# Hongje/OTVM

Measured on AMD Instinct MI355X. Metric: frames_per_sec, higher is better.
Workload: dtype f16x3 (fp32 operands split into fp16 hi+lo, fp32 accumulate); 1 GPU; synthetic 1920x1080 clip, T=140 frames (untimed lead-in 0 + warmup 5 + timed: the last 135), memory every 5, max 5 slots, trimap propagation + alpha + memorize per frame, one sequence per GPU; weights=synthetic (otvm_amd.synth_weights seed 0), parallelism=sequence-per-gpu x1, batch=1

## Files before the change

### include/otvm_hip.h

```cpp
#ifndef OTVM_HIP_H
#define OTVM_HIP_H

#include <stdint.h>

#ifdef __cplusplus
extern "C" {
#endif

#define OTVM_ACT_NONE 0
#define OTVM_ACT_RELU 1
#define OTVM_ACT_LEAKY 2

#define OTVM_PREC_F32 0
#define OTVM_PREC_F16X3 1
#define OTVM_PREC_F16 2

const char* otvm_last_error(void);
#define OTVM_ABI_VERSION 21
int otvm_abi_version(void);

int otvm_pack_conv_weight(const float* w_oihw, int O, int I, int kh, int kw, int ws, const float* scale,
                          float* w_packed, int O_pad, int I_pad, int K_pad, void* stream);

int64_t otvm_patch_weight_bytes_f16x3(int O, int I_pad);
// ... 25 lines not shown
    int tune;
    void* splitk_ws; int64_t splitk_ws_bytes;
    int batch;
    int64_t in_bs, out_bs, res_bs;
    int gn_bs;
    int norm_bs;
    const void* w_wfrag;
    const float* gn_gamma; const float* gn_beta;
    float* gn_scale_out; float* gn_shift_out;
    unsigned* gn_counter;
    int gn_tab_bs;
    int ws_bs;
    const float* res_scale;
    int res_scale_bs;
    const float* in_res; int in_res_ld; int64_t in_res_bs;
} otvm_conv_params;
int otvm_conv2d_accepts_input_residual(const otvm_conv_params* p);

typedef struct otvm_head_params {
    const float* w; const float* b; int n_out;
    const float* img; int img_ld;
    int64_t P;
    float* alpha_out; int alpha_stride;
    float* tri_out;
    float* sm; int sm_ld;
    int64_t img_bs, alpha_bs, tri_bs, sm_bs;
    const void* w16;
} otvm_head_params;
int otvm_conv2d_head(const otvm_conv_params* p, const otvm_head_params* h, void* stream);
int otvm_conv2d_head_fgr(const otvm_conv_params* p, const otvm_head_params* h, float* fgr, int64_t fgr_bs, void* stream);
// ... 249 lines not shown
```

### otvm_amd/csrc/conv_f16x3.hip

```cpp
#include "common.h"
#include <type_traits>
#include <hip/hip_fp16.h>
#include <stdlib.h>

#include "conv_f16x3_kernel.h"

namespace {

#ifndef OTVM_WAVE_PF
#define OTVM_WAVE_PF 3
#endif

template <bool RELU_IN>
__global__ __launch_bounds__(64) void conv_wave_f16x3_kernel(const Conv3Args pa) {
    Conv3Args p = pa;
    {
        const int zb = blockIdx.z;
        p.in += zb * p.in_bs;
        p.out += zb * p.out_bs;
        if (p.residual) p.residual += zb * p.res_bs;
        if (p.gn_stats) p.gn_stats += zb * p.gn_bs;
        p.wscale += zb * p.ws_bs;
        if (p.bias) p.bias += zb * p.ws_bs;
    }
// ... 325 lines not shown
    return 0;
}

extern "C" int64_t otvm_wave_weight_bytes_f16x3(int O_pad, int K_pad) { return (int64_t)O_pad * K_pad * 2 * sizeof(_Float16); }

extern "C" int otvm_pack_wave_weight_f16x3(const void* w_hi, const void* w_lo, int O_pad, int K_pad, void* w_wfrag, void* stream) {
    OTVM_REQUIRE(w_hi && w_lo && w_wfrag && O_pad % 32 == 0 && K_pad % 32 == 0, "otvm_pack_wave_weight_f16x3: bad arguments");
    hipLaunchKernelGGL(pack_wave_weight_kernel, dim3(O_pad / 32), dim3(256), 0, (hipStream_t)stream, (const _Float16*)w_hi,
                       (const _Float16*)w_lo, K_pad, (_Float16*)w_wfrag);
    OTVM_CHECK_LAUNCH("otvm_pack_wave_weight_f16x3");
    return 0;
}

int otvm_conv2d_patch_f16x3_impl(const otvm_conv_params* p, void* stream);

static inline int tune_code(int tile, int S) { return (tile + 1) * 16 + S; }

static int launch_wave(Conv3Args& a, hipStream_t s, int ksplit) {
    a.tiles_m = otvm_ceil_div(a.M, 64);
    a.tiles_n = otvm_ceil_div(a.Cout, 64);
    const dim3 grid(a.tiles_m * a.tiles_n, ksplit, a.batch), block(64);
    if ((int64_t)a.H * a.W * a.in_ld >= (1ll << 31) - (1 << 20)) {
        otvm_set_error("otvm_conv2d(f16x3 wave tile): input view too large for 32-bit offsets");
        return 1;
    }
    if (a.in_relu) hipLaunchKernelGGL((conv_wave_f16x3_kernel<true>), grid, block, 0, s, a);
    else hipLaunchKernelGGL((conv_wave_f16x3_kernel<false>), grid, block, 0, s, a);
    OTVM_CHECK_LAUNCH("otvm_conv2d(f16x3 wave tile)");
    return 0;
}

static int launch_tile(int tile, Conv3Args& a, hipStream_t s, int S) {
    if (a.npass == 1) return otvm_launch_tile_p1(tile, a, s, S);
    if (tile == T64x64W1) return launch_wave(a, s, S);
    if (is_m16_tile(tile)) return otvm_launch_m16_tile(tile - T_M16, a, s, S);
    if (is_glds_tile(tile)) return otvm_launch_glds_tile(tile - T_GLDS, a, s, S);
    return launch_tile_form<false, 3, false>(tile, a, s, S);
}

static bool config_ok(const otvm_conv_params* p, int tile, int S) {
    if (!is_gemm_tile(tile) || S < 1 || S > 8) return false;
    const int64_t M = (int64_t)p->Ho * p->Wo;
    if (TILE_BN(tile) == 256 && !(p->Cout >= 256 && (otvm_ceil_div(p->Cout, 128) & 1) == 0)) return false;
    if (p->in_scale && !(f16x3_fast_layout(p->kh * p->kw, p->Cin) && !p->in_relu && tile != T64x64W1)) return false;
    const int bt = base_tile(tile);
    if ((bt == T256x128W4 || bt == T128x256W4 || bt == T256x256W4) && !f16x3_fast_layout(p->kh * p->kw, p->Cin)) return false;
    if ((bt == T64x64D || bt == T128x64D) && !f16x3_fast_layout(p->kh * p->kw, p->Cin)) return false;
    if (tile == T64x64W1 && !(p->w_wfrag && f16x3_fast_layout(p->kh * p->kw, p->Cin) && (p->in_ld & 3) == 0)) return false;
    if (tile == T64x64W1 && p->res_scale) return false;
    if (p->precision == OTVM_PREC_F16 && (tile == T64x64W1 || tile == T256x256W4 || is_m16_tile(tile))) return false;
    if (is_glds_tile(tile) && !(p->w_wfrag && f16x3_fast_layout(p->kh * p->kw, p->Cin) && (p->in_ld & 3) == 0 &&
                                (int64_t)p->H * p->W * p->in_ld * 4 < (1ll << 31))) return false;
    if (S > 1) {
        const int nchunks = p->K_pad / 32;
        const int ldp = (p->Cout + 3) & ~3;
        if (!p->splitk_ws || nchunks / S < 4) return false;
        const int64_t nb = p->batch > 1 ? p->batch : 1;
        if (nb * S * M * ldp * (int64_t)sizeof(float) > p->splitk_ws_bytes || M * (ldp / 4) >= (1ll << 32)) return false;
    }
    return true;
}

static int run_config(const otvm_conv_params* p, Conv3Args& a, int tile, int S, hipStream_t s) {
    if (S <= 1) return launch_tile(tile, a, s, 1);
    const int64_t M = a.M;
    const int ldp = (p->Cout + 3) & ~3;
    Conv3Args b = a;
    b.out = (float*)p->splitk_ws; b.out_ld = ldp; b.split_stride = M * ldp; b.out_bs = (int64_t)S * M * ldp;
    b.bias = nullptr; b.residual = nullptr; b.res_scale = nullptr; b.act = OTVM_ACT_NONE; b.gn_stats = nullptr; b.tail.scale = nullptr;
    const int rc = launch_tile(tile, b, s, S);
    if (rc) return rc;
    int64_t blocks = (M * (ldp / 4) + 255) / 256;
    if (blocks > 2048) blocks = 2048;
    const int g_batch = a.batch;
    hipLaunchKernelGGL(splitk_finish_kernel, dim3((int)blocks, g_batch), dim3(256), 0, s, (const float*)p->splitk_ws, S,
                       (int64_t)M * ldp, M, p->Cout, ldp, p->bias, p->residual, p->res_ld, p->act, p->out,
                       p->out_ld, a.out_bs, a.res_bs, a.ws_bs, a.res_scale, a.rs_bs);
    OTVM_CHECK_LAUNCH("otvm_conv2d(split-K finish)");
    if (p->gn_stats) {
// ... 26 lines not shown
extern "C" int otvm_conv2d_candidates(const otvm_conv_params* p, int* out, int max_n) {
    int n = 0;
    if (!p || !out || !otvm_prec_is_split(p->precision)) return 0;
    auto add = [&](int code) { if (n < max_n) out[n++] = code; };
    if (otvm_conv2d_stem_eligible(p)) add(tune_code(T_STEM, 1));
    if (otvm_conv2d_patch_eligible(p)) add(tune_code(T_PATCH, 1));
    if (p->in_res) return n;
    const int64_t M = (int64_t)p->Ho * p->Wo;
    const int nchunks = p->K_pad / 32;
    static const int tiles_wide[] = {T256x256, T256x128, T128x128, T128x64, T64x64, T256x128W4, T128x256W4, T64x64W1, T64x64D, T128x64D};
    static const int tiles_64[] = {T256x64, T128x64, T64x64, T64x64W1, T64x64D, T128x64D};
    static const int tiles_32[] = {T256x32, T64x64};
    const int* tl = p->Cout <= 32 ? tiles_32 : (p->Cout <= 64 ? tiles_64 : tiles_wide);
    const int ntl = p->Cout <= 32 ? 2 : (p->Cout <= 64 ? 6 : 10);
    static const int splits[] = {1, 2, 3, 4, 6, 8};
    for (int i = 0; i < ntl; ++i) {
        const int t = tl[i];
        const int64_t wgs = (int64_t)otvm_ceil_div(M, TILE_BM(t)) * otvm_ceil_div(p->Cout, TILE_BN(t));
        if (wgs > 16384 && TILE_BM(t) < 256) continue;
        if (t == T64x64W1 && wgs > 4096) continue;
        for (int j = 0; j < 6; ++j) {
            const int S = splits[j];
            if (S > 1 && (wgs * S > (t == T64x64W1 ? 4096 : 1536) || nchunks < 16)) continue;
            const bool g_ok = glds_mode() != 0 && is_glds_tile(T_GLDS + t) && config_ok(p, T_GLDS + t, S);
            const bool m_ok = g_ok && m16_mode() != 0 && config_ok(p, T_M16 + t, S);
            if (g_ok && !(m_ok && m16_mode() == 2)) add(tune_code(T_GLDS + t, S));
            if (m_ok) add(tune_code(T_M16 + t, S));
            if ((!g_ok || glds_mode() == 2) && config_ok(p, t, S)) add(tune_code(t, S));
        }
    }
    return n;
}

int otvm_conv2d_igemm_accepts_input_norm(const otvm_conv_params* p) {
    return p && otvm_prec_is_split(p->precision) && f16x3_fast_layout(p->kh * p->kw, p->Cin) && !p->in_relu && p->w_hi ? 1 : 0;
}

int otvm_conv2d_f16x3_impl(const otvm_conv_params* p, void* stream) {
    OTVM_REQUIRE(p->w_hi && p->w_lo && p->w_scale, "otvm_conv2d: precision f16x3 needs w_hi / w_lo / w_scale");
    const int forced_tile = p->tune ? p->tune / 16 - 1 : -1, forced_S = p->tune & 15;
    OTVM_REQUIRE(!p->in_res || (otvm_conv2d_patch_eligible(p) && (!p->tune || forced_tile == T_PATCH)),
                 "otvm_conv2d: in_res (identity inside the fused input normalisation) is a patch-kernel feature");
    const bool gemm_only = (p->batch > 1 && p->ws_bs) || (p->residual && p->res_scale);
    OTVM_REQUIRE(!gemm_only || (p->kh == 1 && p->kw == 1), "otvm_conv2d: ws_bs / res_scale are for 1x1 layers (implicit-GEMM route)");
    if (forced_tile == T_STEM || (!p->tune && otvm_conv2d_stem_eligible(p))) {
        OTVM_REQUIRE(otvm_conv2d_stem_eligible(p), "otvm_conv2d: tune asks for the stem kernel on a layer it cannot take");
        return otvm_conv2d_stem_f16x3(p, stream);
    }
    if (p->tune && forced_tile == T_PATCH) {
        OTVM_REQUIRE(otvm_conv2d_patch_eligible(p), "otvm_conv2d: tune asks for the patch kernel on a layer it cannot take");
        return otvm_conv2d_patch_f16x3_forced(p, stream);
    }
    if (!p->tune) {
        const int rc = otvm_conv2d_patch_f16x3_impl(p, stream);
        if (rc != -1) return rc;
    }
    Conv3Args a;
    a.in = p->in; a.wh = (const _Float16*)p->w_hi; a.wl = (const _Float16*)p->w_lo; a.wscale = p->w_scale;
    a.bias = p->bias; a.residual = p->residual; a.out = p->out; a.gn_stats = p->gn_stats;
    a.H = p->H; a.W = p->W; a.Cin = p->Cin; a.in_ld = p->in_ld; a.K_pad = p->K_pad; a.res_ld = p->res_ld;
    a.Ho = p->Ho; a.Wo = p->Wo; a.Cout = p->Cout; a.out_ld = p->out_ld;
    a.kh = p->kh; a.kw = p->kw; a.stride = p->stride; a.pad = p->pad; a.dil = p->dil;
    a.in_relu = p->in_relu; a.act = p->act;
    a.M = p->Ho * p->Wo; a.taps = p->kh * p->kw; a.nchunks = p->K_pad / 32;
    a.split_stride = 0;
    a.wf = (const _Float16*)p->w_wfrag;
    a.npass = p->precision == OTVM_PREC_F16 ? 1 : 3;
    a.tail = otvm_gn_tail_of(p);
    a.in_scale = p->in_scale; a.in_shift = p->in_shift;
    a.in_slope = p->in_act == OTVM_ACT_RELU ? 0.f : (p->in_act == OTVM_ACT_LEAKY ? 0.01f : 1.f);
    a.norm_bs = p->batch > 1 ? p->norm_bs : 0;
    OTVM_REQUIRE(!p->in_scale || otvm_conv2d_igemm_accepts_input_norm(p),
                 "otvm_conv2d: fused input normalisation on the implicit-GEMM path needs Cin %% 32 == 0 and no in_relu");
    const int g_batch = a.batch = p->batch > 1 ? p->batch : 1;
    a.in_bs = g_batch > 1 ? p->in_bs : 0; a.out_bs = g_batch > 1 ? p->out_bs : 0; a.res_bs = g_batch > 1 ? p->res_bs : 0;
    a.gn_bs = g_batch > 1 ? p->gn_bs : 0;
    a.ws_bs = g_batch > 1 ? p->ws_bs : 0;
    a.res_scale = p->residual ? p->res_scale : nullptr; a.rs_bs = g_batch > 1 ? p->res_scale_bs : 0;
    OTVM_REQUIRE(!a.res_scale || (((uintptr_t)a.res_scale & 15) == 0 && (a.rs_bs & 3) == 0 && p->Cout % 4 == 0),
                 "otvm_conv2d: res_scale must be 16-byte aligned");
    hipStream_t s = (hipStream_t)stream;
    const int64_t M = a.M;
    if (p->tune) {
        OTVM_REQUIRE(config_ok(p, forced_tile, forced_S), "otvm_conv2d: tune code %d is not a legal configuration of this layer",
                     p->tune);
        return run_config(p, a, forced_tile, forced_S, s);
    }
    static const int splitk = otvm_probe_int("OTVM_SPLITK", 1);
    static const int min_total = otvm_probe_int("OTVM_SPLITK_MINTOTAL", 32);
    if (splitk && p->splitk_ws && a.nchunks >= min_total) {
        const bool wide = p->Cout > 64;
        const int64_t tiles = (int64_t)otvm_ceil_div(M, 128) * otvm_ceil_div(p->Cout, wide ? 128 : 64);
        int S = (int)(384 / (tiles > 0 ? tiles : 1));
        if (S > 8) S = 8;
        static const int min_chunks = otvm_probe_int("OTVM_SPLITK_MINCHUNKS", 8);
        if (S > a.nchunks / min_chunks) S = a.nchunks / min_chunks;
        if (p->gn_stats && a.nchunks < 256 && tiles > 8) S = 1;
        const int tk = wide ? T128x128 : T128x64;
        while (S >= 2 && !config_ok(p, tk, S)) --S;
        if (tiles < 192 && S >= 2) return run_config(p, a, glds_mode() && config_ok(p, T_GLDS + tk, S) ? (m16_mode() == 2 && config_ok(p, T_M16 + tk, S) ? T_M16 : T_GLDS) + tk : tk, S, s);
    }
    const int use_glds = glds_mode();
    const bool use_m16 = m16_mode() == 2 || (m16_mode() == 1 && M >= m16_min_pixels());
    auto pick = [&](int t) { return use_glds && config_ok(p, T_GLDS + t, 1) ? (use_m16 && config_ok(p, T_M16 + t, 1) ? T_M16 : T_GLDS) + t : t; };
    if (p->Cout <= 32) return launch_tile(pick(T256x32), a, s, 1);
    if (p->Cout <= 64) return launch_tile(pick((M >= 256 * 128) ? T256x64 : T64x64), a, s, 1);
    if (config_ok(p, T256x256, 1)) {
        const int64_t huge = (int64_t)otvm_ceil_div(M, 256) * otvm_ceil_div(p->Cout, 256);
        static const int t_huge = otvm_probe_int("OTVM_T_HUGE", 256);
        if (huge >= t_huge) return launch_tile(pick(T256x256), a, s, 1);
    }
    const int64_t big = (int64_t)otvm_ceil_div(M, 256) * otvm_ceil_div(p->Cout, 128);
    static const int t_big = otvm_probe_int("OTVM_T_BIG", 128);
    if (big >= t_big) return launch_tile(pick(T256x128), a, s, 1);
    const int64_t mid = (int64_t)otvm_ceil_div(M, 128) * otvm_ceil_div(p->Cout, 128);
// ... 8 lines not shown
```

### otvm_amd/csrc/conv_f16x3_kernel.h

```cpp
#pragma once
#pragma clang diagnostic ignored "-Winline-asm"
#include "common.h"
#include "f16x3_ops.h"
#include <type_traits>
#include <hip/hip_fp16.h>
#include <stdlib.h>

#ifndef OTVM_PF_DEPTH
#define OTVM_PF_DEPTH 3
#endif
#ifndef OTVM_PFS_SMALL
#define OTVM_PFS_SMALL 1
#endif
#ifndef OTVM_PFS_MID
#define OTVM_PFS_MID 1
#endif
#ifndef OTVM_PFS_LARGE
#define OTVM_PFS_LARGE 1
#endif
#ifndef OTVM_ABL_NOMFMA
#define OTVM_ABL_NOMFMA 0
#endif
#ifndef OTVM_ABL_NOLOAD
#define OTVM_ABL_NOLOAD 0
// ... 15 lines not shown
struct Conv3Args {
    const float* in; const _Float16* wh; const _Float16* wl; const float* wscale; const float* bias;
    const float* residual; float* out; double* gn_stats;
    int H, W, Cin, in_ld, K_pad, res_ld, Ho, Wo, Cout, out_ld;
    int kh, kw, stride, pad, dil, in_relu, act;
    int M, taps, nchunks, tiles_m, tiles_n;
    int64_t split_stride;
    int64_t in_bs, out_bs, res_bs; int gn_bs;
    const _Float16* wf;
    const float* in_scale; const float* in_shift; float in_slope; int norm_bs;
    OtvmGnTail tail;
    int ws_bs; const float* res_scale; int rs_bs;
    unsigned in_bytes;
    int batch;
    int npass;
};

int otvm_launch_glds_tile(int base, Conv3Args& a, hipStream_t s, int S);
int otvm_launch_m16_tile(int base, Conv3Args& a, hipStream_t s, int S);
int otvm_launch_tile_p1(int tile, Conv3Args& a, hipStream_t s, int S);
int otvm_launch_glds_tile_p1(int base, Conv3Args& a, hipStream_t s, int S);

namespace {

constexpr int BK = 32;
constexpr int LDH = 40;

inline bool f16x3_fast_layout(int taps, int I_pad) { return I_pad % 32 == 0 && taps <= 32; }

template <int BM, int BN, int WM, int WN, bool FAST, bool RELU_IN, bool DB = false, bool NORM_IN = false, bool GLDS = false, int NPASS = 3,
// ... 431 lines not shown
                __syncthreads();
                load_chunk(c + j + PF, rs[j], c + j + PF < c_end);
                compute_ks(0, 0);
                compute_ks(0, 1);
            }
        }
    }
    }

    const int col = lane & 31, rbase = (lane >> 5) * 4;
    auto acc_row = [&](int e) __attribute__((always_inline)) -> int {
        return M16 ? 16 * (e >> 3) + 4 * (lane >> 4) + (e & 3) : (e & 3) + 8 * (e >> 2) + rbase;
    };
    auto acc_col = [&](int e) __attribute__((always_inline)) -> int { return M16 ? 16 * ((e >> 2) & 1) + (lane & 15) : col; };
    __syncthreads();
    const bool vec_ok = ((p.out_ld & 3) == 0) && ((reinterpret_cast<uintptr_t>(outp) & 15) == 0) &&
                        (!p.residual || (((p.res_ld & 3) == 0) && ((reinterpret_cast<uintptr_t>(p.residual) & 15) == 0)));
    const bool interior = vec_ok && m0 + BM <= p.M && n0 + BN <= p.Cout &&
                          !(p.residual && p.res_scale && p.act != OTVM_ACT_RELU);
    auto epilogue_full = [&](auto act_c, auto res_c) __attribute__((always_inline)) {
        constexpr int ACT = decltype(act_c)::value;
        constexpr bool RES = decltype(res_c)::value != 0;
        constexpr bool RSC = decltype(res_c)::value == 2;
        float* patch = reinterpret_cast<float*>(smem) + wave * (32 * 36);
        const int prow = lane >> 3, pc = (lane & 7) * 4;
        f32x4 sc4[TN], bi4[TN];
#pragma unroll
        for (int b = 0; b < TN; ++b) {
            const int n4 = n0 + (wn * TN + b) * 32 + pc;
#pragma unroll
// ... 227 lines not shown
            if (lane < 32 && (lane & (seg - 1)) == 0 && n < p.Cout) {
                const int gl = nl / cg;
                double S, SS;
                otvm_gn_unshift(s, ss, (int)cnt, pil, S, SS);
                atomicAdd(&gred[2 * gl], S);
                atomicAdd(&gred[2 * gl + 1], SS);
            }
        }
        __syncthreads();
        const int ng = (BN + cg - 1) / cg;
        for (int i = threadIdx.x; i < 2 * ng; i += blockDim.x) {
            const int g = n0 / cg + (i >> 1);
            if (g < 32 && gred[i] != 0.0) atomicAdd(&p.gn_stats[2 * g + (i & 1)], gred[i]);
        }
        __syncthreads();
        otvm_gn_table_tail(p.gn_stats, p.M, p.Cout, p.tail, blockIdx.z, gridDim.x * gridDim.y, reinterpret_cast<float*>(gred));
    }
}

template <int BM, int BN, int WM, int WN, bool DB = false, bool FAST_ONLY = false, bool GLDS = false, int NPASS = 3, bool M16T = false>
int launch3(Conv3Args& a, hipStream_t s, int ksplit = 1) {
    a.tiles_m = otvm_ceil_div(a.M, BM);
    a.tiles_n = otvm_ceil_div(a.Cout, BN);
    const dim3 grid(a.tiles_m * a.tiles_n, ksplit, a.batch), block(WM * WN * 64);
    const bool fast = f16x3_fast_layout(a.taps, a.Cin);
    if (fast && (int64_t)a.H * a.W * a.in_ld >= (1ll << 31) - (1 << 20)) {
        otvm_set_error("otvm_conv2d(f16x3): input view too large for 32-bit offsets");
        return 1;
    }
    if (a.in_scale && !(fast && !a.in_relu)) {
        otvm_set_error("otvm_conv2d(f16x3): the fused input normalisation needs a whole-chunk layer (Cin %% 32 == 0) without in_relu");
// ... 94 lines not shown
```

### otvm_amd/engine.py

```python
import ctypes as C
import os

import torch

from . import lib as L

NONE, RELU, LEAKY = 0, 1, 2
GUARD_CLEAR = 2 ** 31 - 1
F16_LIMIT = 65504.0
FUSE_GN_STATS = True
FUSE_GN_APPLY = os.environ.get("OTVM_FUSE_GN_APPLY", "1") != "0"
_GRAPHS_ENV = os.environ.get("OTVM_GRAPHS")
USE_GRAPHS = None if _GRAPHS_ENV in (None, "", "auto") else (_GRAPHS_ENV != "0")
GRAPH_AUTO_PIXELS = 1 << 22


def graphs_wanted(setting, padded_pixels):
    if setting is not None:
        return bool(setting)
    if int(os.environ.get("WORLD_SIZE", "1")) > 1:
        return True
    return padded_pixels < GRAPH_AUTO_PIXELS
PRE_ON_S2 = os.environ.get("OTVM_PRE_ON_S2", "1") != "0"
EVDEC_LATE = os.environ.get("OTVM_EVDEC_LATE", "1") != "0"
# ... 8 lines not shown
FUSE_PPM_HEAD = os.environ.get("OTVM_PPM_HEAD", "1") != "0"
FUSE_GN_PREDICT = os.environ.get("OTVM_GN_PREDICT", "1") != "0"
GN_PREDICT_MIN_PIXELS = int(os.environ.get("OTVM_GN_PREDICT_MIN_PIXELS", "16384"))
GN_PREDICT_PASSES = int(os.environ.get("OTVM_GN_PREDICT_PASSES", "1"))
GN_PREDICT_PLANES = tuple(int(v) for v in os.environ.get("OTVM_GN_PREDICT_PLANES", "64,128,256,512").split(",") if v)
GN_PREDICT_DS = os.environ.get("OTVM_GN_PREDICT_DS", "1") != "0"
GN_PREDICT_KAPPA_P3 = float(os.environ.get("OTVM_GN_PREDICT_KAPPA_P3", "4"))
GN_PREDICT_KAPPA_OFF = float(os.environ.get("OTVM_GN_PREDICT_KAPPA_OFF", "256"))
FUSE_REFINE_TAIL = os.environ.get("OTVM_FUSE_REFINE_TAIL", "0") != "0"
FUSE_HEAD = os.environ.get("OTVM_FUSE_HEAD", "1") != "0"
HEAD16 = os.environ.get("OTVM_HEAD16", "1") != "0"
PPM_ALGEBRA = os.environ.get("OTVM_PPM_ALGEBRA", "1") != "0"


AUTOTUNE = os.environ.get("OTVM_AUTOTUNE", "1") != "0"
_TUNE_CACHE = {}
TUNE_LOG = []
TUNE_FILE = os.environ.get("OTVM_TUNE_FILE")
_TUNE_FILE_LOADED = False


_NON_VARIANT_ENV = ("OTVM_TUNE_FILE", "OTVM_DIST_BACKEND", "OTVM_TEST_FULL_F64", "OTVM_TEST_4K_ORACLE", "OTVM_BENCH_LIVE_PMC",
                    "OTVM_BENCH_FORCE_DIAG", "OTVM_CHECK_FINITE", "OTVM_GRAPHS")


def variant_env():
    return sorted((k, v) for k, v in os.environ.items() if k.startswith("OTVM_") and k not in _NON_VARIANT_ENV)


def kernel_config_digest():
    import hashlib
    return hashlib.sha256(repr((sorted(_TUNE_CACHE.items()), variant_env())).encode()).hexdigest()[:16]


def _tune_file_tag():
    name = "none"
    if torch.cuda.is_available():
        pr = torch.cuda.get_device_properties(torch.cuda.current_device())
        name = "%s/%dcu" % (getattr(pr, "gcnArchName", "?").split(":")[0], pr.multi_processor_count)
    return {"device": name, "abi": L.ABI_VERSION, "variant_env": [list(kv) for kv in variant_env()]}


def _load_tune_file():
    if not (TUNE_FILE and os.path.exists(TUNE_FILE)):
        return
    import json
    import warnings
    try:
        with open(TUNE_FILE) as f:
            doc = json.load(f)
        if not isinstance(doc, dict) or "choices" not in doc:
            raise ValueError("no 'choices' table (file written by an older build)")
        tag = _tune_file_tag()
        if doc.get("abi") != tag["abi"] or (tag["device"] != "none" and doc.get("device") != tag["device"]):
            raise ValueError("tuned for %r / ABI %r, this process runs %r / ABI %r"
                             % (doc.get("device"), doc.get("abi"), tag["device"], tag["abi"]))
        if doc.get("variant_env", []) != tag["variant_env"]:
            raise ValueError("tuned under the switches %r, this process runs under %r" % (doc.get("variant_env", []), tag["variant_env"]))
        for k, v in doc["choices"].items():
            _TUNE_CACHE[tuple(json.loads(k))] = int(v)
    except Exception as e:
        warnings.warn("otvm_amd: ignoring OTVM_TUNE_FILE=%s (%s)" % (TUNE_FILE, e))


def _save_tune_file():
    if not TUNE_FILE:
        return
    import json
    doc = dict(_tune_file_tag())
    doc["choices"] = {json.dumps([int(x) for x in k]): v for k, v in _TUNE_CACHE.items()}
    tmp = "%s.%d.tmp" % (TUNE_FILE, os.getpid())
# ... 138 lines not shown
    v = wg.sum(1).contiguous()
    bs = int(lib.otvm_gram_block(Cin))
    nb = Cin // bs
    blocks = []
    for bi in range(nb):
        rows = wg[:, :, bi * bs:(bi + 1) * bs]
        for bj in range(bi, nb):
            m = torch.einsum("gci,gcj->gij", rows, wg[:, :, bj * bs:(bj + 1) * bs])
            blocks.append((m if bi == bj else 2.0 * m).reshape(32, bs * bs))
    mp = torch.cat(blocks, 1).float().contiguous()
    assert mp.shape[1] == int(lib.otvm_gram_entries(Cin))
    return mp, v


def conv_params(x, cw, out, bias=None, stride=1, pad=0, dil=1, act=NONE, in_relu=0, residual=None, precision=L.PREC_F32,
                in_norm=None, splitk_ws=None):
    Ho = (x.H + 2 * pad - dil * (cw.kh - 1) - 1) // stride + 1
    Wo = (x.W + 2 * pad - dil * (cw.kw - 1) - 1) // stride + 1
    if precision in (L.PREC_F16X3, L.PREC_F16) and cw.w_hi is None:
        raise RuntimeError("otvm_amd: f16x3 convolution requested but the weight was packed without a split")
    return L.ConvParams(x.ptr, x.H, x.W, x.C, x.ld, cw.w.data_ptr(), cw.K_pad,
                        0 if bias is None else bias.data_ptr(),
                        0 if residual is None else residual.ptr, 0 if residual is None else residual.ld,
                        out.ptr, Ho, Wo, cw.O, out.ld, cw.kh, cw.kw, stride, pad, dil, in_relu, act, precision,
                        0 if cw.w_hi is None else cw.w_hi.data_ptr(), 0 if cw.w_lo is None else cw.w_lo.data_ptr(),
                        0 if cw.w_scale is None else cw.w_scale.data_ptr(),
                        0 if cw.w_frag is None else cw.w_frag.data_ptr(), 0,
                        0 if in_norm is None else in_norm[0], 0 if in_norm is None else in_norm[1],
                        0 if in_norm is None else in_norm[2], 0,
                        0 if splitk_ws is None else splitk_ws.data_ptr(),
                        0 if splitk_ws is None else splitk_ws.numel() * splitk_ws.element_size(),
                        x.B, x.bs, out.bs, 0 if residual is None else residual.bs, 0,
                        0 if in_norm is None or len(in_norm) < 4 else in_norm[3],
                        0 if cw.w_wfrag is None else cw.w_wfrag.data_ptr())


class HipEngine:
    def __init__(self, state_dict, device, precision=None):
        self.lib = L.load()
        self.precision_name = precision or default_precision()
        if self.precision_name not in PRECISIONS:
            raise ValueError("otvm_amd: unknown precision %r (choose from %s)" % (self.precision_name, sorted(PRECISIONS)))
        self.precision = PRECISIONS[self.precision_name]
        self.conv_precision = CONV_PRECISIONS[self.precision_name]
        self.dev = torch.device(device)
        if self.dev.type != "cuda":
            raise RuntimeError("otvm_amd: the HIP path needs a GPU device (got %s); there is no CPU fallback" % device)
        self.sd = {k: v.detach().to(self.dev, torch.float32).contiguous() for k, v in state_dict.items()
                   if v.is_floating_point()}
# ... 668 lines not shown
        self._convs = []
        self._predicted = []
        self.diag = None
        self.n_gn = 0
        self.steps = {}
        self._build()
        self.stats_bs = max(self.n_gn, 1) * 64
        self.stats = torch.zeros(self.B * self.stats_bs, dtype=torch.float64, device=self.dev)
        self._bind_stats()
        self.autotune()

    @staticmethod
    def _signature(p):
        return (p.H, p.W, p.Cin, p.in_ld, p.Cout, p.out_ld, p.kh, p.kw, p.stride, p.pad, p.dil, p.in_relu, p.act, int(bool(p.bias)),
                int(bool(p.residual)), p.res_ld, int(bool(p.gn_stats)), int(bool(p.in_scale)), int(bool(p.splitk_ws)), p.precision,
                max(1, p.batch), int(bool(p.res_scale)), int(bool(p.in_res)))

    def _time_conv(self, p, code, stream, reps=3):
        p.tune = code
        fn = self.lib.otvm_conv2d
        self.e.conv_calls += 1 + reps
        L.check(fn(C.byref(p), stream), "autotune warm-up")
        e0, e1 = torch.cuda.Event(enable_timing=True), torch.cuda.Event(enable_timing=True)
        e0.record()
        for _ in range(reps):
            fn(C.byref(p), stream)
        e1.record()
        return e0, e1, reps

    def tune_convs(self, convs):
        if not (AUTOTUNE and self.e.precision == L.PREC_F16X3):
            return
        stream = torch.cuda.current_stream(self.dev).cuda_stream
        codes = (C.c_int * 128)()
        timed_any = False
        for p, name in convs:
            sig = self._signature(p)
            if sig not in _TUNE_CACHE:
                n = int(self.lib.otvm_conv2d_candidates(C.byref(p), codes, 128))
                cands = [0] + [int(codes[i]) for i in range(n)]
                if not WAVE_TILE:
                    cands = [c for c in cands if c // 16 - 1 != 9]
                self._time_conv(p, 0, stream, reps=2)
                timed = [(c,) + self._time_conv(p, c, stream) for c in cands + [0]]
                torch.cuda.synchronize(self.dev)
                ms = {}
                for c, e0, e1, r in timed:
                    t = e0.elapsed_time(e1) / r
                    ms[c] = min(ms.get(c, t), t)
                best = min(ms, key=ms.get)
                if ms[best] > 0.97 * ms[0]:
                    best = 0
                _TUNE_CACHE[sig] = best
                TUNE_LOG.append((name, sig, best, ms))
                timed_any = True
# ... 107 lines not shown
        if key not in self._bufs:
            self._bufs[key] = torch.zeros(n, dtype=dtype, device=self.dev)
        return self._bufs[key]

    def raws(self, name, n, dtype=torch.float32):
        t = self.raw(name, n * self.B, dtype)
        return [t[b * n:(b + 1) * n] for b in range(self.B)]

    def conv(self, S, x, wname, out, stride=1, pad=0, dil=1, act=NONE, in_relu=0, residual=None, in_norm=None, in_res=None,
             up_source=None):
        w = self.e.W[wname]
        assert x.C == w.I_pad, (wname, x.C, w.I_pad)
        Ho = (x.H + 2 * pad - dil * (w.kh - 1) - 1) // stride + 1
        Wo = (x.W + 2 * pad - dil * (w.kw - 1) - 1) // stride + 1
        assert (out.H, out.W) == (Ho, Wo) and out.C >= w.O, (wname, out.H, out.W, Ho, Wo, out.C, w.O)
        p = conv_params(x, w, out, w.bias, stride, pad, dil, act, in_relu, residual, self.e.conv_precision, in_norm, self._ws)
        if in_res is not None:
            assert in_norm is not None and (in_res.H, in_res.W) == (x.H, x.W) and in_res.C >= w.I
            p.in_res, p.in_res_ld, p.in_res_bs = in_res.ptr, in_res.ld, in_res.bs
        self._keep.append(p)
        self._convs.append((p, wname))
        flops = 2 * Ho * Wo * w.O * w.kh * w.kw * w.I * x.B
        abytes = 4 * (x.B * x.H * x.W * w.I * (2 if in_res is not None else 1) + w.O * w.I * w.kh * w.kw
                      + x.B * Ho * Wo * w.O * (2 if residual is not None else 1))
        S.append((self.lib.otvm_conv2d, (C.byref(p),), "conv " + wname, flops, abytes, (x, out.ch(0, _rup(w.O, 4)) if out.C >= _rup(w.O, 4) else out)))
        if up_source is not None:
            assert up_source["out"].t is x.t and up_source["out"].off == x.off and stride == 1 and in_norm is None and in_res is None
            up_source["readers"].append((S, S[-1], p, x, wname))
        return p

    def conv_head(self, S, x, wname, hid_out, head_w, head_b, n_out, img, alpha, alpha_stride, alpha_bs, tri=None, sm=None,
# ... 334 lines not shown
            outs[lname] = x
        return outs["res4"], outs["res3"], outs["res2"]

    def resblock(self, S, x, p, out, tag):
        r = self.buf(tag + "r", x.H, x.W, 256)
        self.conv(S, x, p + ".conv1", r, pad=1, in_relu=1)
        self.conv(S, r, p + ".conv2", out, pad=1, in_relu=1, residual=x)

    def _build(self):
        e, lib = self.e, self.lib
        Hp, Wp, P = self.Hp, self.Wp, self.P
        H2, W2, H4, W4, H8, W8, H16, W16 = Hp // 2, Wp // 2, Hp // 4, Wp // 4, Hp // 8, Wp // 8, Hp // 16, Wp // 16
        self.hw = H16 * W16

        self.SPLITK_WS = [self.raw("splitk_ws%d" % i, (16 << 20) * self.B) for i in range(4)]
        self._ws = self.SPLITK_WS[2]
        self.X11 = self.buf("X11", Hp, Wp, 12)
        self.SQ = self.buf("SQ", Hp, Wp, 4)
        self.SMs = [self.buf("SM0", Hp, Wp, 24), self.buf("SM1", Hp, Wp, 24)]
        self.D80 = self.buf("D80", Hp, Wp, 80)
        self.PROBS_B = self.raws("probs", 3 * P)
        self.CLS_B = self.raws("cls", P, torch.uint8)
        self.ALPHA_P_B = self.raws("alpha_p", P)
        self.TRI_P_B = self.raws("tri_p", 3 * P)
        self.FGR_P_B = self.raws("fgr_p", 3 * P) if self.fgr else None
        self.enc_ws_B = self.raws("enc_ws", _rup(int(lib.otvm_trimap_encode_ws_bytes(Hp, Wp)), 256), torch.uint8)
        self.PROBS, self.CLS, self.ALPHA_P, self.TRI_P = self.PROBS_B[0], self.CLS_B[0], self.ALPHA_P_B[0], self.TRI_P_B[0]

        S = []
        sd = e.sd
# ... 380 lines not shown
```

### otvm_amd/lib.py

```python
import ctypes as C
import os

_HERE = os.path.dirname(os.path.abspath(__file__))
LIB_PATH = os.environ.get("OTVM_HIP_LIB") or os.path.join(_HERE, "libotvm_hip.so")

vp, i32, i64, f32 = C.c_void_p, C.c_int, C.c_int64, C.c_float
PREC_F32, PREC_F16X3, PREC_F16 = 0, 1, 2
ABI_VERSION = 21


class ConvParams(C.Structure):
    _fields_ = [("inp", vp), ("H", i32), ("W", i32), ("Cin", i32), ("in_ld", i32),
                ("w", vp), ("K_pad", i32),
                ("bias", vp),
                ("residual", vp), ("res_ld", i32),
                ("out", vp), ("Ho", i32), ("Wo", i32), ("Cout", i32), ("out_ld", i32),
                ("kh", i32), ("kw", i32), ("stride", i32), ("pad", i32), ("dil", i32),
                ("in_relu", i32), ("act", i32),
                ("precision", i32), ("w_hi", vp), ("w_lo", vp), ("w_scale", vp), ("w_frag", vp),
                ("gn_stats", vp),
                ("in_scale", vp), ("in_shift", vp), ("in_act", i32),
                ("tune", i32),
                ("splitk_ws", vp), ("splitk_ws_bytes", i64),
                ("batch", i32), ("in_bs", i64), ("out_bs", i64), ("res_bs", i64), ("gn_bs", i32), ("norm_bs", i32),
                ("w_wfrag", vp),
                ("gn_gamma", vp), ("gn_beta", vp), ("gn_scale_out", vp), ("gn_shift_out", vp), ("gn_counter", vp), ("gn_tab_bs", i32),
                ("ws_bs", i32), ("res_scale", vp), ("res_scale_bs", i32),
                ("in_res", vp), ("in_res_ld", i32), ("in_res_bs", i64)]


class ConvUpParams(C.Structure):
    _fields_ = [("src", vp), ("Hi", i32), ("Wi", i32), ("Cu", i32), ("src_ld", i32), ("src_bs", i64),
                ("scale", vp), ("shift", vp), ("act", i32), ("norm_bs", i32), ("tile_rows", i32)]


class StmBottleneckParams(C.Structure):
    _fields_ = [("x", vp), ("H", i32), ("W", i32), ("Cin", i32), ("x_ld", i32), ("y", vp), ("y_ld", i32),
                ("w1f", vp), ("w2f", vp), ("w3f", vp), ("s1", vp), ("s2", vp), ("s3", vp), ("b1", vp), ("b2", vp), ("b3", vp),
                ("batch", i32), ("x_bs", i64), ("y_bs", i64), ("tile", i32)]


class GnApplyParams(C.Structure):
    _fields_ = [("x", vp), ("P", i64), ("C", i32), ("ld", i32), ("stats", vp), ("gamma", vp), ("beta", vp),
# ... 193 lines not shown
```

Before: 47.70 frames/s.

## Fuse split-K reduction into conv tile kernel via per-tile tickets

Adds a fused split-K mode: each K-split workgroup writes its partial tile to a per-tile slab, takes an atomic ticket, and the last arriving workgroup sums the slabs and runs the normal epilogue (bias, residual, activation, GN stats). This removes the separate splitk_finish kernel launch and its full-output round trip through memory. Fused variants are added to the autotune candidates and used by default in the heuristic path. The cost is extra atomics, a fence, and a serial reduction done by one workgroup per tile, plus a ticket buffer that must be reset correctly between calls.

```diff
diff --git a/include/otvm_hip.h b/include/otvm_hip.h
--- a/include/otvm_hip.h
+++ b/include/otvm_hip.h
@@ -63,6 +63,7 @@
     const float* res_scale;
     int res_scale_bs;
     const float* in_res; int in_res_ld; int64_t in_res_bs;
+    unsigned* splitk_tickets; int splitk_tickets_n;
 } otvm_conv_params;
 int otvm_conv2d_accepts_input_residual(const otvm_conv_params* p);
 
diff --git a/otvm_amd/csrc/conv_f16x3.hip b/otvm_amd/csrc/conv_f16x3.hip
--- a/otvm_amd/csrc/conv_f16x3.hip
+++ b/otvm_amd/csrc/conv_f16x3.hip
@@ -363,7 +363,9 @@
 
 int otvm_conv2d_patch_f16x3_impl(const otvm_conv_params* p, void* stream);
 
-static inline int tune_code(int tile, int S) { return (tile + 1) * 16 + S; }
+static inline int tune_code(int tile, int S, bool fused = false) { return (tile + 1) * 16 + (fused ? S + 7 : S); }
+static inline int tune_S(int tune) { return (tune & 15) >= 9 ? (tune & 15) - 7 : (tune & 15); }
+static inline bool tune_fused(int tune) { return (tune & 15) >= 9; }
 
 static int launch_wave(Conv3Args& a, hipStream_t s, int ksplit) {
     a.tiles_m = otvm_ceil_div(a.M, 64);
@@ -387,8 +389,9 @@
     return launch_tile_form<false, 3, false>(tile, a, s, S);
 }
 
-static bool config_ok(const otvm_conv_params* p, int tile, int S) {
+static bool config_ok(const otvm_conv_params* p, int tile, int S, bool fused = false) {
     if (!is_gemm_tile(tile) || S < 1 || S > 8) return false;
+    if (fused && (S < 2 || tile == T64x64W1 || TILE_BM(tile) * TILE_BN(tile) >= 256 * 256)) return false;
     const int64_t M = (int64_t)p->Ho * p->Wo;
     if (TILE_BN(tile) == 256 && !(p->Cout >= 256 && (otvm_ceil_div(p->Cout, 128) & 1) == 0)) return false;
     if (p->in_scale && !(f16x3_fast_layout(p->kh * p->kw, p->Cin) && !p->in_relu && tile != T64x64W1)) return false;
@@ -405,13 +408,23 @@
         const int ldp = (p->Cout + 3) & ~3;
         if (!p->splitk_ws || nchunks / S < 4) return false;
         const int64_t nb = p->batch > 1 ? p->batch : 1;
+        if (fused) {
+            const int64_t tiles = (int64_t)otvm_ceil_div(M, TILE_BM(tile)) * otvm_ceil_div(p->Cout, TILE_BN(tile));
+            if (!p->splitk_tickets || nb * tiles > p->splitk_tickets_n) return false;
+            if (nb * tiles * S * TILE_BM(tile) * TILE_BN(tile) * (int64_t)sizeof(float) > p->splitk_ws_bytes) return false;
+        } else
         if (nb * S * M * ldp * (int64_t)sizeof(float) > p->splitk_ws_bytes || M * (ldp / 4) >= (1ll << 32)) return false;
     }
     return true;
 }
 
-static int run_config(const otvm_conv_params* p, Conv3Args& a, int tile, int S, hipStream_t s) {
+static int run_config(const otvm_conv_params* p, Conv3Args& a, int tile, int S, hipStream_t s, bool fused = false) {
     if (S <= 1) return launch_tile(tile, a, s, 1);
+    if (fused) {
+        Conv3Args b = a;
+        b.part = (float*)p->splitk_ws; b.tickets = p->splitk_tickets; b.split_fused = 1;
+        return launch_tile(tile, b, s, S);
+    }
     const int64_t M = a.M;
     const int ldp = (p->Cout + 3) & ~3;
     Conv3Args b = a;
@@ -468,6 +481,7 @@
     const int* tl = p->Cout <= 32 ? tiles_32 : (p->Cout <= 64 ? tiles_64 : tiles_wide);
     const int ntl = p->Cout <= 32 ? 2 : (p->Cout <= 64 ? 6 : 10);
     static const int splits[] = {1, 2, 3, 4, 6, 8};
+    const bool patch_layer = otvm_conv2d_input_norm_kind(p) == 1;
     for (int i = 0; i < ntl; ++i) {
         const int t = tl[i];
         const int64_t wgs = (int64_t)otvm_ceil_div(M, TILE_BM(t)) * otvm_ceil_div(p->Cout, TILE_BN(t));
@@ -476,11 +490,14 @@
         for (int j = 0; j < 6; ++j) {
             const int S = splits[j];
             if (S > 1 && (wgs * S > (t == T64x64W1 ? 4096 : 1536) || nchunks < 16)) continue;
-            const bool g_ok = glds_mode() != 0 && is_glds_tile(T_GLDS + t) && config_ok(p, T_GLDS + t, S);
-            const bool m_ok = g_ok && m16_mode() != 0 && config_ok(p, T_M16 + t, S);
-            if (g_ok && !(m_ok && m16_mode() == 2)) add(tune_code(T_GLDS + t, S));
-            if (m_ok) add(tune_code(T_M16 + t, S));
-            if ((!g_ok || glds_mode() == 2) && config_ok(p, t, S)) add(tune_code(t, S));
+            for (int fused = 0; fused <= (S > 1 && !patch_layer ? 1 : 0); ++fused) {
+                const bool fu = fused != 0;
+                const bool g_ok = glds_mode() != 0 && is_glds_tile(T_GLDS + t) && config_ok(p, T_GLDS + t, S, fu);
+                const bool m_ok = g_ok && m16_mode() != 0 && config_ok(p, T_M16 + t, S, fu);
+                if (g_ok && !(m_ok && m16_mode() == 2)) add(tune_code(T_GLDS + t, S, fu));
+                if (m_ok) add(tune_code(T_M16 + t, S, fu));
+                if ((!g_ok || glds_mode() == 2) && config_ok(p, t, S, fu)) add(tune_code(t, S, fu));
+            }
         }
     }
     return n;
@@ -492,7 +509,8 @@
 
 int otvm_conv2d_f16x3_impl(const otvm_conv_params* p, void* stream) {
     OTVM_REQUIRE(p->w_hi && p->w_lo && p->w_scale, "otvm_conv2d: precision f16x3 needs w_hi / w_lo / w_scale");
-    const int forced_tile = p->tune ? p->tune / 16 - 1 : -1, forced_S = p->tune & 15;
+    const int forced_tile = p->tune ? p->tune / 16 - 1 : -1, forced_S = tune_S(p->tune);
+    const bool forced_fused = tune_fused(p->tune);
     OTVM_REQUIRE(!p->in_res || (otvm_conv2d_patch_eligible(p) && (!p->tune || forced_tile == T_PATCH)),
                  "otvm_conv2d: in_res (identity inside the fused input normalisation) is a patch-kernel feature");
     const bool gemm_only = (p->batch > 1 && p->ws_bs) || (p->residual && p->res_scale);
@@ -518,6 +536,7 @@
     a.in_relu = p->in_relu; a.act = p->act;
     a.M = p->Ho * p->Wo; a.taps = p->kh * p->kw; a.nchunks = p->K_pad / 32;
     a.split_stride = 0;
+    a.part = nullptr; a.tickets = nullptr; a.split_fused = 0;
     a.wf = (const _Float16*)p->w_wfrag;
     a.npass = p->precision == OTVM_PREC_F16 ? 1 : 3;
     a.tail = otvm_gn_tail_of(p);
@@ -536,9 +555,9 @@
     hipStream_t s = (hipStream_t)stream;
     const int64_t M = a.M;
     if (p->tune) {
-        OTVM_REQUIRE(config_ok(p, forced_tile, forced_S), "otvm_conv2d: tune code %d is not a legal configuration of this layer",
+        OTVM_REQUIRE(config_ok(p, forced_tile, forced_S, forced_fused), "otvm_conv2d: tune code %d is not a legal configuration of this layer",
                      p->tune);
-        return run_config(p, a, forced_tile, forced_S, s);
+        return run_config(p, a, forced_tile, forced_S, s, forced_fused);
     }
     static const int splitk = otvm_probe_int("OTVM_SPLITK", 1);
     static const int min_total = otvm_probe_int("OTVM_SPLITK_MINTOTAL", 32);
@@ -549,10 +568,12 @@
         if (S > 8) S = 8;
         static const int min_chunks = otvm_probe_int("OTVM_SPLITK_MINCHUNKS", 8);
         if (S > a.nchunks / min_chunks) S = a.nchunks / min_chunks;
+        const int tk = wide ? T128x128 : T128x64;
+        static const int fuse = otvm_probe_int("OTVM_SPLITK_FUSED", 1);
+        const bool fu = fuse && S >= 2 && config_ok(p, tk, 2, true);
         if (p->gn_stats && a.nchunks < 256 && tiles > 8) S = 1;
-        const int tk = wide ? T128x128 : T128x64;
-        while (S >= 2 && !config_ok(p, tk, S)) --S;
-        if (tiles < 192 && S >= 2) return run_config(p, a, glds_mode() && config_ok(p, T_GLDS + tk, S) ? (m16_mode() == 2 && config_ok(p, T_M16 + tk, S) ? T_M16 : T_GLDS) + tk : tk, S, s);
+        while (S >= 2 && !config_ok(p, tk, S, fu)) --S;
+        if (tiles < 192 && S >= 2) return run_config(p, a, glds_mode() && config_ok(p, T_GLDS + tk, S, fu) ? (m16_mode() == 2 && config_ok(p, T_M16 + tk, S, fu) ? T_M16 : T_GLDS) + tk : tk, S, s, fu);
     }
     const int use_glds = glds_mode();
     const bool use_m16 = m16_mode() == 2 || (m16_mode() == 1 && M >= m16_min_pixels());
diff --git a/otvm_amd/csrc/conv_f16x3_kernel.h b/otvm_amd/csrc/conv_f16x3_kernel.h
--- a/otvm_amd/csrc/conv_f16x3_kernel.h
+++ b/otvm_amd/csrc/conv_f16x3_kernel.h
@@ -53,6 +53,7 @@
     unsigned in_bytes;
     int batch;
     int npass;
+    float* part; unsigned* tickets; int split_fused;
 };
 
 int otvm_launch_glds_tile(int base, Conv3Args& a, hipStream_t s, int S);
@@ -514,6 +515,59 @@
     };
     auto acc_col = [&](int e) __attribute__((always_inline)) -> int { return M16 ? 16 * ((e >> 2) & 1) + (lane & 15) : col; };
     __syncthreads();
+    unsigned gn_wgs = gridDim.x * gridDim.y;
+    if constexpr (BM * BN < 256 * 256)
+    if (p.split_fused) {
+        const int S = gridDim.y;
+        constexpr int SLAB_BYTES = BM * BN * 4, QUADS = TM * TN * 4;
+        const int tile_id = blockIdx.z * gridDim.x + bid;
+        __amdgpu_buffer_rsrc_t prs = otvm_buffer_rsrc(p.part + (int64_t)tile_id * S * (BM * BN), (unsigned)S * SLAB_BYTES);
+        const unsigned own = blockIdx.y * (unsigned)SLAB_BYTES + tid * 16u;
+        otvm_static_for<QUADS>([&](auto i_c) __attribute__((always_inline)) {
+            constexpr int i = decltype(i_c)::value, t = i >> 2, qd = i & 3;
+            const f32x16& c = acc[t / TN][t % TN];
+            const f32x4 v = {c[4 * qd], c[4 * qd + 1], c[4 * qd + 2], c[4 * qd + 3]};
+            __builtin_amdgcn_raw_buffer_store_b128(__builtin_bit_cast(u32x4, v), prs, own + i * (NT * 16), 0, 16);
+        });
+        asm volatile("s_waitcnt vmcnt(0)" ::: "memory");
+        __syncthreads();
+        volatile unsigned* const is_last = reinterpret_cast<volatile unsigned*>(smem);
+        if (tid == 0) {
+            const unsigned drawn = __hip_atomic_fetch_add(p.tickets + tile_id, 1u, __ATOMIC_RELAXED, __HIP_MEMORY_SCOPE_AGENT);
+            if (drawn == (unsigned)S - 1) {
+                __builtin_amdgcn_fence(__ATOMIC_ACQUIRE, "agent");
+                asm volatile("s_waitcnt vmcnt(0)" ::: "memory");
+            }
+            *is_last = drawn == (unsigned)S - 1 ? 1u : 0u;
+        }
+        __syncthreads();
+        if (!*is_last) return;
+        __syncthreads();
+        constexpr int BATCH = QUADS <= 16 ? QUADS : 8;
+        const unsigned mine = tid * 16u;
+        auto add_slab = [&](int z, auto first_c) __attribute__((always_inline)) {
+            constexpr bool FIRST = decltype(first_c)::value;
+            const unsigned zo = z * (unsigned)SLAB_BYTES + mine;
+            otvm_static_for<QUADS / BATCH>([&](auto g_c) __attribute__((always_inline)) {
+                constexpr int g = decltype(g_c)::value;
+                f32x4 v[BATCH];
+#pragma unroll
+                for (int j = 0; j < BATCH; ++j)
+                    v[j] = __builtin_bit_cast(f32x4, (u32x4)__builtin_amdgcn_raw_buffer_load_b128(prs, zo + (g * BATCH + j) * (NT * 16), 0, 16));
+                otvm_static_for<BATCH>([&](auto j_c) __attribute__((always_inline)) {
+                    constexpr int j = decltype(j_c)::value, i = g * BATCH + j, t = i >> 2, qd = i & 3;
+                    f32x16& c = acc[t / TN][t % TN];
+                    if constexpr (FIRST) { c[4 * qd] = v[j].x; c[4 * qd + 1] = v[j].y; c[4 * qd + 2] = v[j].z; c[4 * qd + 3] = v[j].w; }
+                    else { c[4 * qd] += v[j].x; c[4 * qd + 1] += v[j].y; c[4 * qd + 2] += v[j].z; c[4 * qd + 3] += v[j].w; }
+                });
+                __builtin_amdgcn_sched_barrier(0);
+            });
+        };
+        add_slab(0, std::true_type{});
+        for (int z = 1; z < S; ++z) add_slab(z, std::false_type{});
+        if (tid == 0) __hip_atomic_store(p.tickets + tile_id, 0u, __ATOMIC_RELAXED, __HIP_MEMORY_SCOPE_AGENT);
+        gn_wgs = gridDim.x;
+    }
     const bool vec_ok = ((p.out_ld & 3) == 0) && ((reinterpret_cast<uintptr_t>(outp) & 15) == 0) &&
                         (!p.residual || (((p.res_ld & 3) == 0) && ((reinterpret_cast<uintptr_t>(p.residual) & 15) == 0)));
     const bool interior = vec_ok && m0 + BM <= p.M && n0 + BN <= p.Cout &&
@@ -771,7 +825,7 @@
             if (g < 32 && gred[i] != 0.0) atomicAdd(&p.gn_stats[2 * g + (i & 1)], gred[i]);
         }
         __syncthreads();
-        otvm_gn_table_tail(p.gn_stats, p.M, p.Cout, p.tail, blockIdx.z, gridDim.x * gridDim.y, reinterpret_cast<float*>(gred));
+        otvm_gn_table_tail(p.gn_stats, p.M, p.Cout, p.tail, blockIdx.z, gn_wgs, reinterpret_cast<float*>(gred));
     }
 }
 
diff --git a/otvm_amd/engine.py b/otvm_amd/engine.py
--- a/otvm_amd/engine.py
+++ b/otvm_amd/engine.py
@@ -46,6 +46,9 @@
 
 
 AUTOTUNE = os.environ.get("OTVM_AUTOTUNE", "1") != "0"
+SPLITK_FUSED = int(os.environ.get("OTVM_SPLITK_FUSED", "1"))
+SPLITK_TICKETS = 16384
+TUNE_REV = 2
 _TUNE_CACHE = {}
 TUNE_LOG = []
 TUNE_FILE = os.environ.get("OTVM_TUNE_FILE")
@@ -70,7 +73,7 @@
     if torch.cuda.is_available():
         pr = torch.cuda.get_device_properties(torch.cuda.current_device())
         name = "%s/%dcu" % (getattr(pr, "gcnArchName", "?").split(":")[0], pr.multi_processor_count)
-    return {"device": name, "abi": L.ABI_VERSION, "variant_env": [list(kv) for kv in variant_env()]}
+    return {"device": name, "abi": L.ABI_VERSION, "tune_rev": TUNE_REV, "variant_env": [list(kv) for kv in variant_env()]}
 
 
 def _load_tune_file():
@@ -87,6 +90,8 @@
         if doc.get("abi") != tag["abi"] or (tag["device"] != "none" and doc.get("device") != tag["device"]):
             raise ValueError("tuned for %r / ABI %r, this process runs %r / ABI %r"
                              % (doc.get("device"), doc.get("abi"), tag["device"], tag["abi"]))
+        if doc.get("tune_rev", 1) != tag["tune_rev"]:
+            raise ValueError("candidate lists of generation %r, this build offers generation %r" % (doc.get("tune_rev", 1), tag["tune_rev"]))
         if doc.get("variant_env", []) != tag["variant_env"]:
             raise ValueError("tuned under the switches %r, this process runs under %r" % (doc.get("variant_env", []), tag["variant_env"]))
         for k, v in doc["choices"].items():
@@ -255,12 +260,12 @@
 
 
 def conv_params(x, cw, out, bias=None, stride=1, pad=0, dil=1, act=NONE, in_relu=0, residual=None, precision=L.PREC_F32,
-                in_norm=None, splitk_ws=None):
+                in_norm=None, splitk_ws=None, splitk_tickets=None):
     Ho = (x.H + 2 * pad - dil * (cw.kh - 1) - 1) // stride + 1
     Wo = (x.W + 2 * pad - dil * (cw.kw - 1) - 1) // stride + 1
     if precision in (L.PREC_F16X3, L.PREC_F16) and cw.w_hi is None:
         raise RuntimeError("otvm_amd: f16x3 convolution requested but the weight was packed without a split")
-    return L.ConvParams(x.ptr, x.H, x.W, x.C, x.ld, cw.w.data_ptr(), cw.K_pad,
+    p = L.ConvParams(x.ptr, x.H, x.W, x.C, x.ld, cw.w.data_ptr(), cw.K_pad,
                         0 if bias is None else bias.data_ptr(),
                         0 if residual is None else residual.ptr, 0 if residual is None else residual.ld,
                         out.ptr, Ho, Wo, cw.O, out.ld, cw.kh, cw.kw, stride, pad, dil, in_relu, act, precision,
@@ -274,6 +279,9 @@
                         x.B, x.bs, out.bs, 0 if residual is None else residual.bs, 0,
                         0 if in_norm is None or len(in_norm) < 4 else in_norm[3],
                         0 if cw.w_wfrag is None else cw.w_wfrag.data_ptr())
+    if splitk_ws is not None and splitk_tickets is not None:
+        p.splitk_tickets, p.splitk_tickets_n = splitk_tickets.data_ptr(), splitk_tickets.numel()
+    return p
 
 
 class HipEngine:
@@ -972,7 +980,7 @@
     def _signature(p):
         return (p.H, p.W, p.Cin, p.in_ld, p.Cout, p.out_ld, p.kh, p.kw, p.stride, p.pad, p.dil, p.in_relu, p.act, int(bool(p.bias)),
                 int(bool(p.residual)), p.res_ld, int(bool(p.gn_stats)), int(bool(p.in_scale)), int(bool(p.splitk_ws)), p.precision,
-                max(1, p.batch), int(bool(p.res_scale)), int(bool(p.in_res)))
+                max(1, p.batch), int(bool(p.res_scale)), int(bool(p.in_res)), int(bool(p.splitk_tickets)))
 
     def _time_conv(self, p, code, stream, reps=3):
         p.tune = code
@@ -990,13 +998,26 @@
         if not (AUTOTUNE and self.e.precision == L.PREC_F16X3):
             return
         stream = torch.cuda.current_stream(self.dev).cuda_stream
-        codes = (C.c_int * 128)()
+        codes = (C.c_int * 256)()
         timed_any = False
         for p, name in convs:
             sig = self._signature(p)
             if sig not in _TUNE_CACHE:
-                n = int(self.lib.otvm_conv2d_candidates(C.byref(p), codes, 128))
+                n = int(self.lib.otvm_conv2d_candidates(C.byref(p), codes, 256))
                 cands = [0] + [int(codes[i]) for i in range(n)]
+                if SPLITK_FUSED == 2 and any(c % 16 >= 9 for c in cands):
+                    cands = [c for c in cands if c % 16 >= 9]
+                    self._time_conv(p, cands[0], stream, reps=2)
+                    timed = [(c,) + self._time_conv(p, c, stream) for c in cands]
+                    torch.cuda.synchronize(self.dev)
+                    ms = {}
+                    for c, e0, e1, r in timed:
+                        ms[c] = e0.elapsed_time(e1) / r
+                    _TUNE_CACHE[sig] = min(ms, key=ms.get)
+                    TUNE_LOG.append((name, sig, _TUNE_CACHE[sig], ms))
+                    timed_any = True
+                    p.tune = _TUNE_CACHE[sig]
+                    continue
                 if not WAVE_TILE:
                     cands = [c for c in cands if c // 16 - 1 != 9]
                 self._time_conv(p, 0, stream, reps=2)
@@ -1134,7 +1155,8 @@
         Ho = (x.H + 2 * pad - dil * (w.kh - 1) - 1) // stride + 1
         Wo = (x.W + 2 * pad - dil * (w.kw - 1) - 1) // stride + 1
         assert (out.H, out.W) == (Ho, Wo) and out.C >= w.O, (wname, out.H, out.W, Ho, Wo, out.C, w.O)
-        p = conv_params(x, w, out, w.bias, stride, pad, dil, act, in_relu, residual, self.e.conv_precision, in_norm, self._ws)
+        p = conv_params(x, w, out, w.bias, stride, pad, dil, act, in_relu, residual, self.e.conv_precision, in_norm, self._ws,
+                        self._ws_tickets.get(self._ws.data_ptr()) if self._ws is not None else None)
         if in_res is not None:
             assert in_norm is not None and (in_res.H, in_res.W) == (x.H, x.W) and in_res.C >= w.I
             p.in_res, p.in_res_ld, p.in_res_bs = in_res.ptr, in_res.ld, in_res.bs
@@ -1499,6 +1521,8 @@
         self.hw = H16 * W16
 
         self.SPLITK_WS = [self.raw("splitk_ws%d" % i, (16 << 20) * self.B) for i in range(4)]
+        self._ws_tickets = {t.data_ptr(): self.raw("splitk_tickets%d" % i, SPLITK_TICKETS * self.B, torch.int32)
+                            for i, t in enumerate(self.SPLITK_WS)} if SPLITK_FUSED else {}
         self._ws = self.SPLITK_WS[2]
         self.X11 = self.buf("X11", Hp, Wp, 12)
         self.SQ = self.buf("SQ", Hp, Wp, 4)
diff --git a/otvm_amd/lib.py b/otvm_amd/lib.py
--- a/otvm_amd/lib.py
+++ b/otvm_amd/lib.py
@@ -26,7 +26,8 @@
                 ("w_wfrag", vp),
                 ("gn_gamma", vp), ("gn_beta", vp), ("gn_scale_out", vp), ("gn_shift_out", vp), ("gn_counter", vp), ("gn_tab_bs", i32),
                 ("ws_bs", i32), ("res_scale", vp), ("res_scale_bs", i32),
-                ("in_res", vp), ("in_res_ld", i32), ("in_res_bs", i64)]
+                ("in_res", vp), ("in_res_ld", i32), ("in_res_bs", i64),
+                ("splitk_tickets", vp), ("splitk_tickets_n", i32)]
 
 
 class ConvUpParams(C.Structure):
```

Measured after the change: 47.66 frames/s. About the same (-0.1%).
